# YufengJin/torch_renderer

Measured on AMD Instinct MI355X. Metric: frames/sec fwd+bwd, 512×512, ~6k-face mesh, batch=64; 1/2/4/8 MI355X, higher is better.
Workload: dtype f32; 1 GPU; cow (F=5856, V=2930), 512x512, 64 views/GPU, fwd+bwd: depth+silhouette+Phong RGB from one raster pass, grads to verts and per-view R,t; mesh=cow, H=512, W=512, views_per_gpu=64, global_views=64, parallelism=view-sharded x1

## Files before the change

torch_renderer_amd/csrc/mr_tile_raster.h:

```cpp
#pragma once

struct TileCols {
  float C0, C1;
  float omax;
};
MR_DEV TileCols tile_cols(int x0, int H, int W) {
  TileCols t;
  t.C1 = W > H ? 0.5f * (float)H : 0.5f * (float)W;
  t.C0 = 0.5f * (float)W - 0.5f - (float)x0;
  t.omax = (float)max(W, H) / (float)min(W, H);
  return t;
}
MR_DEV unsigned long long rect_mask(int rx0, int rx1, int ry0, int ry1) {
  const unsigned long long row = (2ull << rx1) - (1ull << rx0);
  const unsigned long long rows = (0x0101010101010101ull >> (8 * (7 - ry1))) & (~0ull << (8 * ry0));
  return row * rows;
}
MR_DEV unsigned long long tri_mask(const FaceRec& r, const float* ys, int rx0, int rx1, int ry0, int ry1,
                                   const TileCols& tc) {
  const float s = r.area > 0.0f ? 1.0f : -1.0f;
  float Gx[3], K[3], rA[3], ax[3], sC1[3], sC0[3];
  bool up[3];
  const float vx[3] = {r.x0, r.x1, r.x2}, vy[3] = {r.y0, r.y1, r.y2};
#pragma unroll
  for (int i = 0; i < 3; ++i) {
    const int a = (i + 1) % 3, b = (i + 2) % 3;
    const float dx = vx[b] - vx[a], dy = vy[b] - vy[a];
    const float A = s * dy;
    const float tol = 1e-6f * (fabsf(dx) + fabsf(dy)) * (tc.omax + fabsf(vx[a]) + fabsf(vy[a]));
    Gx[i] = s * dx;
    K[i] = Gx[i] * vy[a] + 2.0f * tol;
    up[i] = A >= 0.0f;
    rA[i] = A != 0.0f ? __builtin_amdgcn_rcpf(A) : 1e30f;
    ax[i] = vx[a];
    sC1[i] = up[i] ? -tc.C1 : tc.C1;
    sC0[i] = (up[i] ? tc.C0 : -tc.C0) + 0.02f;
  }
  unsigned long long m = 0;
#pragma unroll
  for (int ry = 0; ry < MR_TS; ++ry) {
    if (ry < ry0 || ry > ry1) continue;
    const float py = ys[ry];
    int hi = rx1, lo = rx0;
#pragma unroll
    for (int i = 0; i < 3; ++i) {
      const float T = fmaf(fmaf(Gx[i], py, -K[i]), rA[i], ax[i]);
      const float v = __builtin_amdgcn_fmed3f(fmaf(T, sC1[i], sC0[i]), -10.0f, 10.0f);
      const int h = (int)floorf(v);
      if (up[i]) hi = min(hi, h);
      else lo = max(lo, -h);
    }
    if (lo <= hi) m |= ((2ull << hi) - (1ull << lo)) << (8 * ry);
  }
  return m;
}

MR_DEV int kth_bit(unsigned long long m, int k) {
  const unsigned lo = (unsigned)m;
  const int clo = __popc(lo);
  const bool hi = k >= clo;
  unsigned x = hi ? (unsigned)(m >> 32) : lo;
  int pos = hi ? 32 : 0;
  k = hi ? k - clo : k;
#pragma unroll
  for (int sh = 16; sh >= 1; sh >>= 1) {
    const int c = __popc(x & ((1u << sh) - 1u));
    const bool go = k >= c;
    x = go ? x >> sh : x;
    k = go ? k - c : k;
    pos = go ? pos + sh : pos;
  }
  return pos;
}

MR_DEV bool frag_depth(const FaceRec& r, float x, float y, float pad, bool persp, bool clipb, bool fast, float& pz,
                       bool& inside) {
  if (x > r.xmax + pad || x < r.xmin - pad || y > r.ymax + pad || y < r.ymin - pad) return false;
  const float e0 = edge_fn(x, y, r.x1, r.y1, r.x2, r.y2);
  const float e1 = edge_fn(x, y, r.x2, r.y2, r.x0, r.y0);
  const float e2 = edge_fn(x, y, r.x0, r.y0, r.x1, r.y1);
  if (fast) {
    const bool inp = (e0 > 0.0f) & (e1 > 0.0f) & (e2 > 0.0f);
    const bool inn = (e0 < 0.0f) & (e1 < 0.0f) & (e2 < 0.0f);
    if (!(r.area > 0.0f ? inp : inn)) return false;
  }
  const float w0 = e0 / r.area, w1 = e1 / r.area, w2 = e2 / r.area;
  float c0, c1, c2, b0, b1, b2;
  if (persp) persp_fwd(w0, w1, w2, r.z0, r.z1, r.z2, c0, c1, c2);
  else { c0 = w0; c1 = w1; c2 = w2; }
  if (clipb) clip_fwd(c0, c1, c2, b0, b1, b2);
  else { b0 = c0; b1 = c1; b2 = c2; }
  pz = b0 * r.z0 + b1 * r.z1 + b2 * r.z2;
  if (pz < 0.0f) return false;
  inside = c0 > 0.0f && c1 > 0.0f && c2 > 0.0f;
  return true;
}

MR_DEV bool frag_keep(const FaceRec& r, float x, float y, float pad, float blur, bool persp, bool clipb,
                      bool fast, float& pz) {
  bool inside;
  if (!frag_depth(r, x, y, pad, persp, clipb, fast, pz, inside)) return false;
  if (!inside) {
    if (!(blur > 0.0f)) return false;
    if (pt_tri_dist(x, y, r) >= blur) return false;
  }
  return true;
}

#define MR_NONE 0x7fffffff

MR_DEV unsigned rec_code(int id, int64_t NF) {
  return id < NF ? 2u * (unsigned)id : 2u * (unsigned)(id - NF) + 1u;
}
MR_DEV int code_rec(unsigned code, int64_t NF) {
  return (code & 1u) ? (int)(NF + (code >> 1)) : (int)(code >> 1);
}
MR_DEV int rec_orig(int id, int64_t NF) { return id >= NF ? (int)(id - NF) : id; }

MR_DEV bool pair_keep(const FaceRec* __restrict__ recs, int64_t NF, int id, const FaceRec& r, float x, float y,
                      float pad, float blur, bool persp, bool clipb, int& cid, float& pz) {
  const bool second = id >= NF;
  const int oid = second ? (int)(id - NF) : (int)(id + NF);
  const FaceRec ro = recs[oid];
  const FaceRec& r1 = second ? ro : r;
  const FaceRec& r2 = second ? r : ro;
  const int id1 = second ? oid : id, id2 = second ? id : oid;
  FragEval e1, e2;
  const bool k1 = (r1.flags & FR_VALID) && eval_face(r1, x, y, pad, blur, persp, clipb, e1);
  const bool k2 = (r2.flags & FR_VALID) && eval_face(r2, x, y, pad, blur, persp, clipb, e2);
  if (k1 && k2) {
    const bool use2 = fabsf(e2.sdist) < fabsf(e1.sdist);
    cid = use2 ? id2 : id1;
    pz = use2 ? e2.pz : e1.pz;
    return true;
  }
  if (k1 || k2) {
    cid = k1 ? id1 : id2;
    pz = k1 ? e1.pz : e2.pz;
    return true;
  }
  return false;
}

struct StageRecs {
  float rec[16][64];
};
MR_DEV void stage_rec_put(StageRecs& S, int lane, const FaceRec& r) {
  const float* f = (const float*)&r;
#pragma unroll
  for (int i = 0; i < 16; ++i) S.rec[i][lane] = f[i];
}
MR_DEV FaceRec stage_rec_get(const StageRecs& S, int m) {
  FaceRec r;
  float* f = (float*)&r;
#pragma unroll
  for (int i = 0; i < 16; ++i) f[i] = S.rec[i][m];
  return r;
}
MR_DEV unsigned long long frag_key(float z, int f) {
  const unsigned zb = z == 0.0f ? 0u : __float_as_uint(z);
  return ((unsigned long long)zb << 32) | (unsigned)f;
}

struct FwdParams {
  int N, H, W, TX, T, K;
  float blur, bbox_pad;
  int persp, clipb;
  const int64_t* view_first;
  int64_t F;
  int64_t NF;
  const ClipRec* crec;
  const FaceRec* recs;
  const int* list;
  const int4* units;
  const int64_t* view_count;
  const int* cnt;
  const int* start;
  const int* vbase;
  int64_t list_cap;
  int mfpb;
  int fill;
  int emit_frag;
  int fill_first;
  int* ctr;
  unsigned long long* tkey;
  int* tdone;
  int* sface;
  const int* stile;
  int64_t* p2f;
  float* zbuf;
  float* bary;
  float* dists;
  ShadeParams S;
  const ShadeRec* srec;
  int out_flags;
  float* depth;
  float* sil;
  float* rgb;
  int32_t* p2f32;
  float4* frec;
  int* sgrp;
  uint8_t* sgpix;
  float isig;
  int4* sent;
  float4* spix;
  const int* sorder;
  int* sorder_ws;
  int4* units_ws2;
};

struct WaveStage {
  StageRecs rec;
  int id[64];
  int meta[64];
  int mark[64];
  unsigned long long key[64];
  unsigned long long cmask[64];
  float xs[MR_TS], ys[MR_TS];
};

struct Bg {
  float d, s, c[4];
};
template <int MODE>
MR_DEV Bg background(const FwdParams& P) {
  Bg b;
  b.d = b.s = -1.0f;
  b.c[0] = b.c[1] = b.c[2] = b.c[3] = -1.0f;
  if (MODE == 1) {
    PixGeom G;
    ShadeOut o;
    ShadeCache C;
    shade_fwd(P.S, 0, false, G, 0.f, 0.f, 0.f, 0.f, 0.f, o, C);
    b.d = o.depth;
    b.s = o.sil;
    b.c[0] = o.rgb[0]; b.c[1] = o.rgb[1]; b.c[2] = o.rgb[2]; b.c[3] = o.alpha;
  }
  return b;
}

template <int MODE, int CH>
MR_DEV void fill_chunk(const FwdParams& P, const Bg& b, int n, int c, bool vec) {
  const int lane = threadIdx.x & 63;
  const int64_t HW = (int64_t)P.H * P.W * (MODE == 0 ? P.K : 1);
  if (MODE == 0 && vec) {
    const int64_t q0 = (int64_t)c * 64;
    const int nq = (int)min((int64_t)64, HW / 4 - q0);
    if (nq <= 0) return;
    const int64_t pix = (int64_t)n * HW + 4 * q0;
    const float4 m1 = make_float4(-1.f, -1.f, -1.f, -1.f);
    const longlong2 l1 = make_longlong2(-1ll, -1ll);
    fill_words<2>((longlong2*)(P.p2f + pix), nq, lane, l1);
    fill_words<1>((float4*)(P.zbuf + pix), nq, lane, m1);
    fill_words<1>((float4*)(P.dists + pix), nq, lane, m1);
    fill_words<3>((float4*)(P.bary + pix * 3), nq, lane, m1);
  } else if (vec) {
    const int64_t g = (int64_t)c * 64 + lane;
    if (g >= HW / 4) return;
    const int64_t pix = (int64_t)n * HW + 4 * g;
    if (MODE == 0) {
      const float4 m1 = make_float4(-1.f, -1.f, -1.f, -1.f);
      longlong2* q = (longlong2*)(P.p2f + pix);
      q[0] = make_longlong2(-1ll, -1ll);
      q[1] = make_longlong2(-1ll, -1ll);
      *(float4*)(P.zbuf + pix) = m1;
      *(float4*)(P.dists + pix) = m1;
      float4* q3 = (float4*)(P.bary + pix * 3);
      q3[0] = m1; q3[1] = m1; q3[2] = m1;
    } else {
      if (P.out_flags & MR_OUT_DEPTH) *(float4*)(P.depth + pix) = make_float4(b.d, b.d, b.d, b.d);
      if (P.out_flags & MR_OUT_SIL) {
        if (P.out_flags & MR_OUT_SIL_RGBA) {
          float4* q = (float4*)(P.sil + pix * 4);
          const float4 v = make_float4(1.0f, 1.0f, 1.0f, b.s);
          q[0] = v; q[1] = v; q[2] = v; q[3] = v;
        } else {
          *(float4*)(P.sil + pix) = make_float4(b.s, b.s, b.s, b.s);
        }
      }
      if (P.p2f32) *(int4*)(P.p2f32 + pix) = make_int4(-1, -1, -1, -1);
      if (P.out_flags & MR_OUT_RGB) {
        float4* q = (float4*)(P.rgb + pix * CH);
        if (CH == 4) {
          const float4 v = make_float4(b.c[0], b.c[1], b.c[2], b.c[3]);
          q[0] = v; q[1] = v; q[2] = v; q[3] = v;
        } else {
          float r0 = b.c[0], g0 = b.c[1], b0 = b.c[2], r1 = r0, g1 = g0, b1 = b0, r2 = r0, g2 = g0, b2 = b0;
          asm volatile("" : "+v"(r1), "+v"(g1), "+v"(b1), "+v"(r2), "+v"(g2), "+v"(b2));
          q[0] = make_float4(r0, g0, b0, r1);
          q[1] = make_float4(g1, b1, r2, g2);
          q[2] = make_float4(b2, r0, g0, b0);
        }
      }
    }
  } else {
    const int64_t i = (int64_t)c * 64 + lane;
    if (i >= HW) return;
    const int64_t q = (int64_t)n * HW + i;
    if (MODE == 0) {
      P.p2f[q] = -1ll;
      P.zbuf[q] = -1.0f;
      P.dists[q] = -1.0f;
      for (int k = 0; k < 3; ++k) P.bary[q * 3 + k] = -1.0f;
    } else {
      if (P.out_flags & MR_OUT_DEPTH) P.depth[q] = b.d;
      if (P.out_flags & MR_OUT_SIL) {
        if (P.out_flags & MR_OUT_SIL_RGBA) *(float4*)(P.sil + q * 4) = make_float4(1.0f, 1.0f, 1.0f, b.s);
        else P.sil[q] = b.s;
      }
      if (P.p2f32) P.p2f32[q] = -1;
      if (P.out_flags & MR_OUT_RGB)
        for (int k = 0; k < CH; ++k) P.rgb[q * CH + k] = b.c[k];
    }
  }
}

MR_DEV void fill_frag_unlisted(const FwdParams& P, int n, int c) {
  const int lane = threadIdx.x & 63;
  const int64_t HW = (int64_t)P.H * P.W;
  const int64_t q0 = (int64_t)c * 64;
  const int nq = (int)min((int64_t)64, HW / 4 - q0);
  if (nq <= 0) return;
  bool listed = false;
  if (lane < nq) {
    const int p0 = (int)(4 * q0);
    int y = p0 / P.W, x = p0 - y * P.W + 4 * lane;
    while (x >= P.W) {
      x -= P.W;
      ++y;
    }
    listed = P.cnt[(int64_t)n * P.T + (y >> 3) * P.TX + (x >> 3)] > 0;
  }
  const unsigned long long lm = __ballot(listed);
  const int64_t pix = (int64_t)n * HW + 4 * q0;
  const float4 m1 = make_float4(-1.f, -1.f, -1.f, -1.f);
  longlong2* p2 = (longlong2*)(P.p2f + pix);
  float4* pz = (float4*)(P.zbuf + pix);
  float4* pd = (float4*)(P.dists + pix);
  float4* pb = (float4*)(P.bary + pix * 3);
#pragma unroll
  for (int k = 0; k < 2; ++k) {
    const int j = k * 64 + lane;
    if (j < 2 * nq && !((lm >> (j >> 1)) & 1ull)) p2[j] = make_longlong2(-1ll, -1ll);
  }
  if (lane < nq && !((lm >> lane) & 1ull)) {
    pz[lane] = m1;
    pd[lane] = m1;
  }
#pragma unroll
  for (int k = 0; k < 3; ++k) {
    const int j = k * 64 + lane;
    if (j < 3 * nq && !((lm >> (j / 3)) & 1ull)) pb[j] = m1;
  }
}

MR_DEV void fill_chunk_render_lc(const FwdParams& P, const Bg& b, int n, int c, int CH) {
  const int lane = threadIdx.x & 63;
  const int64_t HW = (int64_t)P.H * P.W;
  const int64_t q0 = (int64_t)c * 64;
  const int nq = (int)min((int64_t)64, HW / 4 - q0);
  if (nq <= 0) return;
  const int64_t pix = (int64_t)n * HW + 4 * q0;
  if (P.out_flags & MR_OUT_DEPTH) fill_words<1>((float4*)(P.depth + pix), nq, lane, make_float4(b.d, b.d, b.d, b.d));
  if (P.out_flags & MR_OUT_SIL) {
    if (P.out_flags & MR_OUT_SIL_RGBA) fill_words<4>((float4*)(P.sil + pix * 4), nq, lane, make_float4(1.0f, 1.0f, 1.0f, b.s));
    else fill_words<1>((float4*)(P.sil + pix), nq, lane, make_float4(b.s, b.s, b.s, b.s));
  }
  if (P.p2f32) fill_words<1>((int4*)(P.p2f32 + pix), nq, lane, make_int4(-1, -1, -1, -1));
  if (P.out_flags & MR_OUT_RGB) {
    float4* q = (float4*)(P.rgb + pix * CH);
    if (CH == 4) {
      fill_words<4>(q, nq, lane, make_float4(b.c[0], b.c[1], b.c[2], b.c[3]));
    } else {
      const float4 w0 = make_float4(b.c[0], b.c[1], b.c[2], b.c[0]);
      const float4 w1 = make_float4(b.c[1], b.c[2], b.c[0], b.c[1]);
      const float4 w2 = make_float4(b.c[2], b.c[0], b.c[1], b.c[2]);
#pragma unroll
      for (int k = 0; k < 3; ++k) {
        const int j = k * 64 + lane;
        if (j < 3 * nq) q[j] = (j % 3) == 0 ? w0 : (j % 3) == 1 ? w1 : w2;
      }
    }
  }
}

template <int MODE, int CH>
__global__ void __launch_bounds__(256) k_fill(FwdParams P) {
  const int gw = blockIdx.x * 4 + (threadIdx.x >> 6), G = gridDim.x * 4;
  const bool vec = (P.W & 3) == 0;
  const int64_t HW = (int64_t)P.H * P.W * (MODE == 0 ? P.K : 1);
  const int cpv = (int)(vec ? (HW / 4 + 63) / 64 : (HW + 63) / 64);
  const int nchunks = P.N * cpv;
  const Bg bg = background<MODE>(P);
#pragma unroll 1
  for (int c = gw; c < nchunks; c += G) {
    if (MODE == 1 && vec) fill_chunk_render_lc(P, bg, c / cpv, c - (c / cpv) * cpv, CH);
    else fill_chunk<MODE, CH>(P, bg, c / cpv, c - (c / cpv) * cpv, vec);
  }
}


#ifdef MR_XP_BV_STAMP
#define MR_XP_BV_WGS 4096
__device__ unsigned long long g_bv_stamp[MR_XP_BV_WGS * 8];
#endif
template <int MODE, int CH>
__global__ void __launch_bounds__(1024) k_bin_view(ViewBinParams P, FwdParams F) {
#ifdef MR_XP_BV_STAMP
  const unsigned long long xp_t0 = __builtin_amdgcn_s_memrealtime();
  const int xp_role = (int)blockIdx.x < P.nviews * P.bands ? 0 : (int)blockIdx.x < P.nviews * P.bands + P.nsrec_wg ? 1 : 2;
  struct XpEnd {
    unsigned long long t0;
    int role;
    __device__ ~XpEnd() {
      __syncthreads();
      const unsigned long long t1 = __builtin_amdgcn_s_memrealtime();
      const int i = (int)threadIdx.x;
      if (blockIdx.x < MR_XP_BV_WGS && i < 8)
        g_bv_stamp[(size_t)blockIdx.x * 8 + i] = i == 0 ? t0 : i == 1 ? t1 : i == 2 ? (unsigned long long)role
                                               : role == 0 ? g_bv_ph[i - 3] : 0ull;
    }
  } xp_end{xp_t0, xp_role};
#endif
  const int b = (int)blockIdx.x - P.nviews * P.bands - P.nsrec_wg;
  if (b < 0) {
    bin_view_body(P);
    return;
  }
  const int nbw = ((int)gridDim.x - P.nviews * P.bands - P.nsrec_wg) * 16;
  const bool vec = (F.W & 3) == 0;
  const int64_t HW = (int64_t)F.H * F.W * (MODE == 0 ? F.K : 1);
  const int cpv = (int)(vec ? (HW / 4 + 63) / 64 : (HW + 63) / 64);
  const Bg bg = background<MODE>(F);
  const int c0 = b * 16 + (int)(threadIdx.x >> 6);
  const int gn = nbw / cpv, gc = nbw - gn * cpv;
  int cn = c0 / cpv, cc = c0 - cn * cpv;
#pragma unroll 1
  for (int c = c0; c < F.fill_first; c += nbw) {
    fill_chunk<MODE, CH>(F, bg, cn, cc, vec);
    cn += gn;
    cc += gc;
    if (cc >= cpv) { cc -= cpv; ++cn; }
  }
}

__attribute__((noinline)) __device__ void raster_pair_rect(const FaceRec* __restrict__ recs, int64_t NF,
                                                           const StageRecs& srec, const int* sid, const float* xs,
                                                           const float* ys, unsigned long long* key, int lane,
                                                           int prect, float pad, float blur, bool persp, bool clipb) {
  const FaceRec r = stage_rec_get(srec, lane);
  const int id = sid[lane];
  for (int yy = (prect >> 6) & 7; yy <= ((prect >> 9) & 7); ++yy)
    for (int xx = prect & 7; xx <= ((prect >> 3) & 7); ++xx) {
      float pz;
      int cid;
      if (pair_keep(recs, NF, id, r, xs[xx], ys[yy], pad, blur, persp, clipb, cid, pz))
        atomicMin(&key[yy * MR_TS + xx], frag_key(pz, (int)rec_code(cid, NF)));
    }
}

#ifndef MR_TR_BGFIRST_FRAG
#define MR_TR_BGFIRST_FRAG 4
#endif
#ifndef MR_RASTER_WAVES
#define MR_RASTER_WAVES 4
#endif
template <int MODE, int CH, bool CLIP>
__global__ void __launch_bounds__(256, MR_RASTER_WAVES) k_tile_raster(FwdParams P) {
  __shared__ WaveStage stage[4];
  const int lane = threadIdx.x & 63;
  const int wave = __builtin_amdgcn_readfirstlane(threadIdx.x >> 6);
  WaveStage& S = stage[wave];
  const int nunits = P.ctr[CTR_UNITS];
  const float pad = P.bbox_pad, blur = P.blur;
  const bool persp = P.persp != 0, clipb = P.clipb != 0;
  const bool fast_ok = !(blur > 0.0f);
  const int H = P.H, W = P.W;
  const int gw = blockIdx.x * 4 + wave, G = gridDim.x * 4;
  const bool vec = (W & 3) == 0;
  const int64_t HW = (int64_t)H * W * (MODE == 0 ? P.K : 1);
  const int cpv = (int)(vec ? (HW / 4 + 63) / 64 : (HW + 63) / 64);
  const int nchunks = P.fill ? P.N * cpv : 0;
  const int parts = (gridDim.x & 7) == 0 ? 8 : 1;
  const int jw = (blockIdx.x / parts) * 4 + wave, Gp = (gridDim.x / parts) * 4;
  const int Cp = (nunits + parts - 1) / parts;
  const int ub = (blockIdx.x % parts) * Cp, ue = ub + Cp < nunits ? ub + Cp : nunits;
  const Bg bg = background<MODE>(P);
  int chunk = P.fill_first + gw;
  auto background_chunks = [&]() {
    const int gn = G / cpv, gc = G - gn * cpv;
    int cn = chunk / cpv, cc = chunk - cn * cpv;
    if (MODE == 0 && P.emit_frag) {
#pragma unroll 1
      for (; chunk < nchunks; chunk += G) {
        fill_frag_unlisted(P, cn, cc);
        cn += gn;
        cc += gc;
        if (cc >= cpv) { cc -= cpv; ++cn; }
      }
    } else {
#pragma unroll 1
      for (; chunk < nchunks; chunk += G) {
        fill_chunk<MODE, CH>(P, bg, cn, cc, vec);
        cn += gn;
        cc += gc;
        if (cc >= cpv) { cc -= cpv; ++cn; }
      }
    }
  };
  if (MODE == 0 && MR_TR_BGFIRST_FRAG > 0 &&
      (blockIdx.x + wave) % (MR_TR_BGFIRST_FRAG > 0 ? MR_TR_BGFIRST_FRAG : 1) == 0)
    background_chunks();
  const int lz = lane_zero();
  const int ulast = max(ue - 1, 0);
  int4 U1v = P.units[min(ub + jw, ulast) + lz];
  int4 U2v = P.units[min(ub + jw + Gp, ulast) + lz];
  int4 U3v = P.units[min(ub + jw + 2 * Gp, ulast) + lz];
  int id1 = P.list[(ub + jw < ue && U1v.y >= 0 && lane < U1v.z) ? U1v.y + lane : 0];
  int id2 = P.list[(ub + jw + Gp < ue && U2v.y >= 0 && lane < U2v.z) ? U2v.y + lane : 0];
  FaceRec r1 = load_rec(P.recs, (ub + jw < ue && U1v.y >= 0 && lane < U1v.z) ? id1 : 0);
#pragma unroll 1
  for (int u = ub + jw; u < ue; u += Gp) {
    const int4 U = make_int4(__builtin_amdgcn_readfirstlane(U1v.x), __builtin_amdgcn_readfirstlane(U1v.y),
                             __builtin_amdgcn_readfirstlane(U1v.z), __builtin_amdgcn_readfirstlane(U1v.w));
    const int id0 = id1;
    const int n = U.x / P.T, t = U.x - n * P.T;
    const int ty = t / P.TX, tx = t - ty * P.TX;
    const int x0 = tx * MR_TS, y0 = ty * MR_TS;
    const TileCols tc = tile_cols(x0, H, W);
    if (lane < MR_TS) S.xs[lane] = col_ndc(x0 + lane < W ? x0 + lane : W - 1, H, W);
    else if (lane < 2 * MR_TS) S.ys[lane - MR_TS] = row_ndc(y0 + lane - MR_TS < H ? y0 + lane - MR_TS : H - 1, H, W);
    S.key[lane] = MR_KEY_EMPTY;
    S.mark[lane] = -1;
    const bool ovf = U.y < 0;
    wave_lds_sync();
#pragma unroll 1
    for (int eb = 0; eb < U.z; eb += 64) {
      const int e = eb + lane;
      int prect = 0;
      unsigned long long cmask = 0;
      if (e < U.z) {
        int id;
        FaceRec r;
        if (ovf) {
          const int64_t vfirst = P.view_first ? P.view_first[n] : (int64_t)n * P.F;
          id = (int)(vfirst + e);
          r = P.recs[id];
        } else {
          id = id0;
          r = r1;
        }
        float bx0 = r.xmin, bx1 = r.xmax, by0 = r.ymin, by1 = r.ymax;
        bool bvalid = (r.flags & FR_VALID) != 0;
        if (CLIP && ovf && (r.flags & FR_PAIR)) {
          const FaceRec ro = P.recs[P.NF + id];
          if (ro.flags & FR_VALID) {
            bx0 = bvalid ? smin(bx0, ro.xmin) : ro.xmin;
            bx1 = bvalid ? smax(bx1, ro.xmax) : ro.xmax;
            by0 = bvalid ? smin(by0, ro.ymin) : ro.ymin;
            by1 = bvalid ? smax(by1, ro.ymax) : ro.ymax;
            bvalid = true;
          }
        }
        int cx0, cx1, cy0, cy1;
        ndc_range_to_pix(bx0 - pad, bx1 + pad, W, H, cx0, cx1);
        ndc_range_to_pix(by0 - pad, by1 + pad, H, W, cy0, cy1);
        cx0 = cx0 > x0 ? cx0 : x0;
        cx1 = cx1 < x0 + MR_TS - 1 ? cx1 : x0 + MR_TS - 1;
        cy0 = cy0 > y0 ? cy0 : y0;
        cy1 = cy1 < y0 + MR_TS - 1 ? cy1 : y0 + MR_TS - 1;
        if (bvalid && cx0 <= cx1 && cy0 <= cy1) {
          if (CLIP && (r.flags & FR_PAIR)) {
            prect = 0x1000 | (cx0 - x0) | ((cx1 - x0) << 3) | ((cy0 - y0) << 6) | ((cy1 - y0) << 9);
          } else {
            const int rx0 = cx0 - x0, rx1 = cx1 - x0, ry0 = cy0 - y0, ry1 = cy1 - y0;
            const bool tm = fast_ok && (r.flags & FR_FAST) &&
                            fmaxf(fmaxf(fabsf(r.xmin), fabsf(r.xmax)), fmaxf(fabsf(r.ymin), fabsf(r.ymax))) < 1e12f;
            cmask = tm ? tri_mask(r, S.ys, rx0, rx1, ry0, ry1, tc) : rect_mask(rx0, rx1, ry0, ry1);
          }
        }
        stage_rec_put(S.rec, lane, r);
        S.id[lane] = id;
      }
      if (eb == 0) {
        r1 = load_rec(P.recs, (u + Gp < ue && U2v.y >= 0 && lane < U2v.z) ? id2 : 0);
        id1 = id2;
        U1v = U2v;
        id2 = P.list[(u + 2 * Gp < ue && U3v.y >= 0 && lane < U3v.z) ? U3v.y + lane : 0];
        U2v = U3v;
        U3v = P.units[min(u + 3 * Gp, ulast) + lz];
      }
      const int np = __popcll(cmask);
      const int pincl = wave_incl_sum(np);
      const int pexcl = pincl - np;
      const int NP = __builtin_amdgcn_readlane(pincl, 63);
      S.meta[lane] = pexcl;
      S.cmask[lane] = cmask;
#pragma unroll 1
      for (int pb = 0; pb < NP; pb += 64) {
        wave_lds_sync();
        if (np > 0 && pexcl > pb && pexcl < pb + 64) S.mark[pexcl - pb] = lane;
        const unsigned long long own = __ballot(np > 0 && pexcl <= pb);
        const int straddle = 63 - __builtin_clzll(own);
        wave_lds_sync();
        int m = S.mark[lane];
        S.mark[lane] = -1;
        if (lane == 0) m = straddle;
        m = wave_incl_max(m);
        const int q = pb + lane;
        if (q < NP) {
          const int p = kth_bit(S.cmask[m], q - S.meta[m]);
          const int sx = p & 7, sy = p >> 3;
          const FaceRec r = stage_rec_get(S.rec, m);
          float pz;
          if (frag_keep(r, S.xs[sx], S.ys[sy], pad, blur, persp, clipb, fast_ok && (r.flags & FR_FAST), pz))
            atomicMin(&S.key[p], frag_key(pz, CLIP ? (int)rec_code(S.id[m], P.NF) : 2 * S.id[m]));
        }
      }
      if (CLIP && __builtin_expect(__ballot(prect != 0) != 0ull, 0)) {
        if (prect) raster_pair_rect(P.recs, P.NF, S.rec, S.id, S.xs, S.ys, S.key, lane, prect, pad, blur, persp, clipb);
      }
      wave_lds_sync();
    }
    unsigned long long k = S.key[lane];
    const int slot = U.w & 0x7fffffff;
    bool emit = true;
    if (U.w < 0) {
      unsigned long long* dst = P.tkey + (int64_t)slot * 64 + lane;
      atomicMin(dst, k);
      asm volatile("s_waitcnt vmcnt(0)" ::: "memory");
      int left = 0;
      if (lane == 0) left = __hip_atomic_fetch_add(&P.tdone[slot], -1, __ATOMIC_RELAXED, __HIP_MEMORY_SCOPE_AGENT);
      left = __builtin_amdgcn_readfirstlane(left);
      emit = left == 0;
      if (emit) k = atomicMin(dst, MR_KEY_EMPTY);
    }
    if (emit) {
      const unsigned code = (unsigned)(k & 0xffffffffull);
      const int px = x0 + (lane & 7), py = y0 + (lane >> 3);
      const bool hit = code != MR_NONE && px < W && py < H;
      const int rid = hit ? (CLIP ? code_rec(code, P.NF) : (int)(code >> 1)) : -1;
      if (MODE == 0 && P.emit_frag) {
        if (px < W && py < H) {
          const int64_t q = (int64_t)n * H * W + (int64_t)py * W + px;
          int64_t f = -1;
          float z = -1.0f, d = -1.0f, b0 = -1.0f, b1 = -1.0f, b2 = -1.0f;
          if (hit) {
            const FaceRec r = load_rec(P.recs, rid);
            FragEval ev;
            eval_face(r, S.xs[lane & 7], S.ys[lane >> 3], pad, blur, persp, clipb, ev);
            if (r.flags & FR_CLIP) clip_unconvert(P.crec[rid], ev.b0, ev.b1, ev.b2, ev.b0, ev.b1, ev.b2);
            f = rec_orig(rid, P.NF); z = ev.pz; d = ev.sdist; b0 = ev.b0; b1 = ev.b1; b2 = ev.b2;
          }
          P.p2f[q] = f;
          P.zbuf[q] = z;
          P.dists[q] = d;
          P.bary[3 * q + 0] = b0;
          P.bary[3 * q + 1] = b1;
          P.bary[3 * q + 2] = b2;
        }
      } else {
        P.sface[(int64_t)slot * 64 + lane] = rid;
      }
    }
    wave_lds_sync();
  }
  background_chunks();
}

__global__ void __launch_bounds__(256) k_shade_rec(ShadeParams S, int64_t F, ShadeRec* __restrict__ out) {
  const int64_t f = (int64_t)blockIdx.x * blockDim.x + threadIdx.x;
  if (f >= F) return;
  ShadeRec R;
  make_shade_rec(S, (uint32_t)f, R);
  out[f] = R;
}

__global__ void __launch_bounds__(256) k_setup_zero(const float* __restrict__ verts, int64_t V,
                                                    const int32_t* __restrict__ faces, const int32_t* __restrict__ ptr,
                                                    const int32_t* __restrict__ adj, float* __restrict__ vn,
                                                    float* __restrict__ vraw, int64_t vb, int* __restrict__ zero,
                                                    int64_t nzero) {
  if ((int64_t)blockIdx.x < vb) {
    const int64_t v = (int64_t)blockIdx.x * blockDim.x + threadIdx.x;
    if (v < V) vertex_normal(verts, faces, ptr, adj, v, vn, vraw);
    return;
  }
  const int64_t base = ((int64_t)blockIdx.x - vb) * 1024;
#pragma unroll
  for (int k = 0; k < 4; ++k) {
    const int64_t i = base + k * 256 + threadIdx.x;
    if (i < nzero) zero[i] = 0;
  }
}

MR_DEV void xcd_slot_range(int nslots, int wave, int& s0, int& step, int& end) {
  const int parts = (gridDim.x & 7) == 0 ? 8 : 1;
  const int per = (nslots + parts - 1) / parts;
  const int x = blockIdx.x % parts;
  const int b = x * per;
  end = b + per < nslots ? b + per : nslots;
  s0 = b + (int)(blockIdx.x / parts) * 4 + wave;
  step = (int)(gridDim.x / parts) * 4;
}

MR_DEV int sort_slot_pixels(int& f, int lane, int* lperm) {
  unsigned long long rem = ~0ull;
  int pos = 0, base = 0;
  while (rem) {
    const int l = (int)__builtin_ctzll(rem);
    const int key = __builtin_amdgcn_readlane(f, l);
    const unsigned long long m = __ballot(f == key);
    const int below = (int)__builtin_amdgcn_mbcnt_hi((unsigned)(m >> 32), __builtin_amdgcn_mbcnt_lo((unsigned)m, 0u));
    pos = f == key ? base + below : pos;
    base += __popcll(m);
    rem &= ~m;
  }
  lperm[pos] = lane;
  wave_lds_sync();
  const int src = lperm[lane];
  f = __builtin_amdgcn_ds_bpermute(src << 2, f);
  wave_lds_sync();
  return src;
}

template <int MODE, int CH>
__global__ void __launch_bounds__(256) k_shade(FwdParams P) {
  __shared__ int lperm[MODE == 1 ? 4 : 1][64];
  const int lane = threadIdx.x & 63;
  const int wave = __builtin_amdgcn_readfirstlane(threadIdx.x >> 6);
  const int nslots = P.ctr[CTR_SLOTS];
  if (nslots <= 0) return;
  const int64_t HW = (int64_t)P.H * P.W;
  int s0, G, send;
  xcd_slot_range(nslots, wave, s0, G, send);
  const int lz = lane_zero();
  const int slast = max(nslots - 1, 0);
  int sc = min(s0, slast);
  int gt_c = P.stile[sc + lz], f_c = P.sface[(int64_t)sc * 64 + lane];
  sc = min(s0 + G, slast);
  int gt_n = P.stile[sc + lz], f_n = P.sface[(int64_t)sc * 64 + lane];
  int p_c = MODE == 1 ? sort_slot_pixels(f_c, lane, lperm[wave]) : lane;
  FaceRec r_c = load_rec(P.recs, f_c < 0 ? 0 : f_c);
  for (int s = s0; s < send; s += G) {
    const int gt = __builtin_amdgcn_readfirstlane(gt_c);
    const int f = f_c, p = p_c;
    const FaceRec r = r_c;
    gt_c = gt_n;
    f_c = f_n;
    if (MODE == 1) p_c = sort_slot_pixels(f_c, lane, lperm[wave]);
    r_c = load_rec(P.recs, f_c < 0 ? 0 : f_c);
    sc = min(s + 2 * G, slast);
    gt_n = P.stile[sc + lz];
    f_n = P.sface[(int64_t)sc * 64 + lane];
    if (MODE == 1) {
      P.sgrp[(int64_t)s * 64 + lane] = f;
      P.sgpix[(int64_t)s * 64 + lane] = (uint8_t)p;
    }
    if (f < 0) continue;
    const int n = gt / P.T, t = gt - n * P.T;
    const int ty = t / P.TX, tx = t - ty * P.TX;
    const int px = tx * MR_TS + (p & 7), py = ty * MR_TS + (p >> 3);
    const int64_t q = n * HW + (int64_t)py * P.W + px;
    const int fo = rec_orig(f, P.NF);
    PixGeom G;
    if (MODE == 1) load_geom(P.srec, (uint32_t)(fo - n * P.F), G);
    FragEval ev;
    const bool hit = eval_face(r, col_ndc(px, P.H, P.W), row_ndc(py, P.H, P.W), P.bbox_pad, P.blur, P.persp,
                               P.clipb, ev);
    if (!hit) continue;
    if (r.flags & FR_CLIP) {
      const ClipRec cr = P.crec[f];
      clip_unconvert(cr, ev.b0, ev.b1, ev.b2, ev.b0, ev.b1, ev.b2);
    }
    if (MODE == 0) {
      P.p2f[q] = (int64_t)fo;
      P.zbuf[q] = ev.pz;
      P.dists[q] = ev.sdist;
      P.bary[3 * q + 0] = ev.b0;
      P.bary[3 * q + 1] = ev.b1;
      P.bary[3 * q + 2] = ev.b2;
    } else {
      P.frec[(int64_t)s * 64 + p] = make_float4(ev.b0, ev.b1, ev.b2, ev.sdist);
      ShadeOut o;
      ShadeCache C;
      shade_fwd(P.S, n, true, G, ev.b0, ev.b1, ev.b2, ev.pz, ev.sdist, o, C);
      if (P.out_flags & MR_OUT_DEPTH) P.depth[q] = o.depth;
      if (P.out_flags & MR_OUT_SIL) {
        if (P.out_flags & MR_OUT_SIL_RGBA) *(float4*)(P.sil + q * 4) = make_float4(1.0f, 1.0f, 1.0f, o.sil);
        else P.sil[q] = o.sil;
      }
      if (P.out_flags & MR_OUT_RGB) {
        P.rgb[q * CH + 0] = o.rgb[0];
        P.rgb[q * CH + 1] = o.rgb[1];
        P.rgb[q * CH + 2] = o.rgb[2];
        if (CH == 4) P.rgb[q * CH + 3] = o.alpha;
      }
      if (P.p2f32) P.p2f32[q] = fo;
    }
  }
}

template <int CH, int SPEC>
__global__ void __launch_bounds__(256) k_shade_render(FwdParams P) {
  __shared__ int lperm[4][64];
  const int lane = threadIdx.x & 63;
  const int wave = __builtin_amdgcn_readfirstlane(threadIdx.x >> 6);
  const int nslots = P.ctr[CTR_SLOTS];
  if (nslots <= 0) return;
  const int64_t HW = (int64_t)P.H * P.W;
  int s0, G, send;
  xcd_slot_range(nslots, wave, s0, G, send);
  const int lz = lane_zero();
  const int slast = max(nslots - 1, 0);
  int sc = min(s0, slast);
  int gt_c = P.stile[sc + lz], f_c = P.sface[(int64_t)sc * 64 + lane];
  sc = min(s0 + G, slast);
  int gt_n = P.stile[sc + lz], f_n = P.sface[(int64_t)sc * 64 + lane];
  int p_c = sort_slot_pixels(f_c, lane, lperm[wave]);
  FaceRec r_c = load_rec(P.recs, f_c < 0 ? 0 : f_c);
  const int of = SPEC ? (MR_OUT_DEPTH | MR_OUT_SIL | MR_OUT_RGB) : P.out_flags;
  int s_prev = -1, f_prev = -1, p_prev = 0, fo_prev = 0;
  bool w_prev = false;
  int64_t q_prev = 0;
  float4 fr_prev = make_float4(0.f, 0.f, 0.f, 0.f);
  ShadeOut o_prev;
  o_prev.depth = o_prev.sil = o_prev.alpha = 0.f;
  o_prev.rgb[0] = o_prev.rgb[1] = o_prev.rgb[2] = 0.f;
  auto store_prev = [&]() {
    if (s_prev < 0) return;
    P.sgrp[(int64_t)s_prev * 64 + lane] = f_prev;
    P.sgpix[(int64_t)s_prev * 64 + lane] = (uint8_t)p_prev;
    if (w_prev) {
      P.frec[(int64_t)s_prev * 64 + p_prev] = fr_prev;
      if (of & MR_OUT_DEPTH) P.depth[q_prev] = o_prev.depth;
      if (of & MR_OUT_SIL) {
        if (!SPEC && (of & MR_OUT_SIL_RGBA)) *(float4*)(P.sil + q_prev * 4) = make_float4(1.0f, 1.0f, 1.0f, o_prev.sil);
        else P.sil[q_prev] = o_prev.sil;
      }
      if (of & MR_OUT_RGB) {
        P.rgb[q_prev * CH + 0] = o_prev.rgb[0];
        P.rgb[q_prev * CH + 1] = o_prev.rgb[1];
        P.rgb[q_prev * CH + 2] = o_prev.rgb[2];
        if (CH == 4) P.rgb[q_prev * CH + 3] = o_prev.alpha;
      }
      if (!SPEC && P.p2f32) P.p2f32[q_prev] = fo_prev;
    }
  };
  for (int s = s0; s < send; s += G) {
    const int gt = __builtin_amdgcn_readfirstlane(gt_c);
    const int f = f_c, p = p_c;
    const FaceRec r = r_c;
    const int n = gt / P.T, t = gt - n * P.T;
    const int ty = t / P.TX, tx = t - ty * P.TX;
    const int px = tx * MR_TS + (p & 7), py = ty * MR_TS + (p >> 3);
    const int64_t q = n * HW + (int64_t)py * P.W + px;
    const int fo = f >= 0 ? (int)rec_orig(f, P.NF) : 0;
    PixGeom Gm;
    load_geom(P.srec, f >= 0 ? (uint32_t)(fo - n * P.F) : 0u, Gm);
    gt_c = gt_n;
    f_c = f_n;
    p_c = sort_slot_pixels(f_c, lane, lperm[wave]);
    r_c = load_rec(P.recs, f_c < 0 ? 0 : f_c);
    sc = min(s + 2 * G, slast);
    gt_n = P.stile[sc + lz];
    f_n = P.sface[(int64_t)sc * 64 + lane];
    store_prev();
    FragEval ev;
    const bool hit = f >= 0 && eval_face(r, col_ndc(px, P.H, P.W), row_ndc(py, P.H, P.W), P.bbox_pad, P.blur,
                                         P.persp, P.clipb, ev);
    ShadeOut o;
    o.depth = o.sil = o.alpha = 0.f;
    o.rgb[0] = o.rgb[1] = o.rgb[2] = 0.f;
    if (hit) {
      if (r.flags & FR_CLIP) {
        const ClipRec cr = P.crec[f];
        clip_unconvert(cr, ev.b0, ev.b1, ev.b2, ev.b0, ev.b1, ev.b2);
      }
      ShadeCache C;
      shade_fwd<SPEC>(P.S, n, true, Gm, ev.b0, ev.b1, ev.b2, ev.pz, ev.sdist, o, C);
    }
    s_prev = s;
    f_prev = f;
    p_prev = p;
    w_prev = hit;
    q_prev = q;
    fo_prev = fo;
    fr_prev = make_float4(ev.b0, ev.b1, ev.b2, ev.sdist);
    o_prev = o;
  }
  store_prev();
}

template <typename K>
static int resident_grid(K kernel, int threads, int fallback_per_cu) {
  int dev = 0, cus = 0, per = 0;
  (void)hipGetDevice(&dev);
  if (hipDeviceGetAttribute(&cus, hipDeviceAttributeMultiprocessorCount, dev) != hipSuccess || cus <= 0) cus = 256;
  if (hipOccupancyMaxActiveBlocksPerMultiprocessor(&per, kernel, threads, 0) != hipSuccess || per <= 0)
    per = fallback_per_cu;
  return cus * per;
}

static FwdParams make_fwd(const mr_raster_settings_t* s, const BinGeom& g, const RasterWS& w, int64_t N,
                          const int64_t* view_first, int64_t F, int64_t NF) {
  FwdParams P;
  memset(&P, 0, sizeof(P));
  P.N = (int)N; P.H = s->H; P.W = s->W; P.TX = g.TX; P.T = g.T; P.K = s->faces_per_pixel;
  P.blur = s->blur_radius;
  P.bbox_pad = sqrtf(s->blur_radius);
  P.persp = s->perspective_correct;
  P.clipb = s->clip_barycentric_coords;
  P.view_first = view_first; P.F = F; P.NF = NF; P.crec = w.crec;
  P.recs = w.recs; P.list = w.list; P.units = w.units; P.ctr = w.ctr; P.tkey = w.tkey;
  P.cnt = w.cnt; P.start = w.start; P.vbase = w.vbase; P.list_cap = g.list_cap; P.mfpb = g.mfpb;
  P.tdone = w.tdone; P.sface = w.sface; P.stile = w.stile;
  P.frec = w.frec;
  P.sgrp = w.sgrp;
  P.sgpix = w.sgpix;
  P.sorder_ws = w.sorder;
  P.units_ws2 = w.units2;
  return P;
}


#ifndef MR_UNIT_ORDER
#define MR_UNIT_ORDER 1
#endif
#ifndef MR_UNIT_ORDER_MIN_VIEWS
#define MR_UNIT_ORDER_MIN_VIEWS 16
#endif
MR_DEV int unit_key(const int4& U) { return U.y < 0 ? 0 : MR_UE + 1 - min(max(U.z, 1), MR_UE); }
__global__ void __launch_bounds__(1024) k_unit_order(const int4* __restrict__ units, const int* __restrict__ ctr,
                                                     int4* __restrict__ out) {
  __shared__ int hist[128];
  const int t = threadIdx.x, n = ctr[CTR_UNITS];
  const int per = (n + 7) / 8, b = (int)blockIdx.x * per, e = min(b + per, n);
  if (t < 128) hist[t] = 0;
  __syncthreads();
  for (int u = b + t; u < e; u += 1024) atomicAdd(&hist[unit_key(units[u])], 1);
  __syncthreads();
  if (t < 64) {
    const int x = hist[2 * t], y = hist[2 * t + 1];
    const int incl = wave_incl_sum(x + y);
    hist[2 * t] = b + incl - (x + y);
    hist[2 * t + 1] = b + incl - y;
  }
  __syncthreads();
  for (int u = b + t; u < e; u += 1024) {
    const int4 U = units[u];
    out[atomicAdd(&hist[unit_key(U)], 1)] = U;
  }
}

static int shade_grid(int64_t slots_cap, int resident) {
  const int sg = (int)(slots_cap / 4 + 1 < resident ? slots_cap / 4 + 1 : resident);
  return (sg + 7) / 8 * 8;
}

#ifndef MR_SHADE_RENDER
#define MR_SHADE_RENDER 1
#endif
template <int CH>
static int launch_shade_render(const FwdParams& P, int64_t slots_cap, hipStream_t st) {
  static int g0 = 0, g1 = 0;
  if (!g0) g0 = resident_grid(k_shade_render<CH, 0>, 256, 4);
  if (!g1) g1 = resident_grid(k_shade_render<CH, 1>, 256, 4);
  const bool spec = drop_in_shading(P.S, CH, P.out_flags) && !P.p2f32 &&
                    P.out_flags == (MR_OUT_DEPTH | MR_OUT_SIL | MR_OUT_RGB);
  const int sg = shade_grid(slots_cap, spec ? g1 : g0);
  return launch(KID_SHADE_RENDER, "k_shade_render", spec ? k_shade_render<CH, 1> : k_shade_render<CH, 0>, sg, 256, 0, st, P);
}

template <int MODE, int CH>
static int launch_raster_and_shade(FwdParams P, const BinGeom& g, int64_t N, hipStream_t st, bool clip) {
  P.fill = 1;
  static int rgrid = 0, rgrid_c = 0, sgrid = 0;
  if (!rgrid) rgrid = resident_grid(k_tile_raster<MODE, CH, false>, 256, 7);
  if (!rgrid_c) rgrid_c = resident_grid(k_tile_raster<MODE, CH, true>, 256, 7);
  if (!sgrid) sgrid = resident_grid(k_shade<MODE, CH>, 256, 6);
  if (MR_UNIT_ORDER && MODE == 1 && P.units_ws2 && N >= MR_UNIT_ORDER_MIN_VIEWS) {
    if (int rc = launch(KID_UNIT_ORDER, "k_unit_order", k_unit_order, 8, 1024, 0, st, P.units, P.ctr, P.units_ws2)) return rc;
    P.units = P.units_ws2;
  }
  if (int rc = launch(KID_TILE_RASTER, "k_tile_raster", clip ? k_tile_raster<MODE, CH, true> : k_tile_raster<MODE, CH, false>,
                      clip ? rgrid_c : rgrid, 256, 0, st, P))
    return rc;
  if (MODE == 0 && P.emit_frag) return MR_OK;
  const int64_t slots_cap = N * (int64_t)g.T;
  if (MODE == 1 && MR_SHADE_RENDER) return launch_shade_render<CH>(P, slots_cap, st);
  return launch(MODE == 0 ? KID_SHADE_FRAG : KID_SHADE_RENDER, "k_shade", k_shade<MODE, CH>, shade_grid(slots_cap, sgrid), 256, 0,
                st, P);
}

template <int CH>
static int launch_fill_and_shade(const FwdParams& P, int64_t slots_cap, hipStream_t st) {
  static int fgrid = 0, sgrid = 0;
  if (!fgrid) fgrid = resident_grid(k_fill<1, CH>, 256, 8);
  if (!sgrid) sgrid = resident_grid(k_shade<1, CH>, 256, 6);
  if (int rc = launch(KID_FILL_FRAG, "k_fill", k_fill<1, CH>, fgrid, 256, 0, st, P)) return rc;
  return launch(KID_SHADE_RENDER, "k_shade", k_shade<1, CH>, shade_grid(slots_cap, sgrid), 256, 0, st, P);
}
```

Measured before the change: 336,500 frames/s.

## Interleave background fill chunks into tile raster loop for render mode

Adds a BGQ variant of the tile raster kernel that writes one background fill chunk (depth, silhouette, packed RGB) per raster unit iteration, instead of leaving all background chunks to a loop after rasterization. The aim is to overlap the store-bound background fill with the compute- and latency-bound rasterization so the memory system stays busy while waves raster. It also adds an optional vmcnt-based pacing hook for background stores, disabled by default. The risk is extra stores and register pressure inside the hot raster loop, and leftover chunks are still handled by the existing tail fill.

```diff
diff --git a/torch_renderer_amd/csrc/mr_tile_raster.h b/torch_renderer_amd/csrc/mr_tile_raster.h
--- a/torch_renderer_amd/csrc/mr_tile_raster.h
+++ b/torch_renderer_amd/csrc/mr_tile_raster.h
@@ -384,6 +384,36 @@
   }
 }
 
+#ifndef MR_BG_INFLIGHT
+#define MR_BG_INFLIGHT 0
+#endif
+template <int MODE>
+MR_DEV void bg_pace() {
+  constexpr int cap = MR_BG_INFLIGHT;
+  if (cap > 0) {
+    constexpr int n = (MODE == 0 ? 7 : 5) * (cap > 0 ? cap - 1 : 0);
+    asm volatile("s_waitcnt vmcnt(%0)" ::"n"(n < 63 ? n : 63) : "memory");
+  }
+}
+
+MR_DEV void fill_chunk_static(const FwdParams& P, const Bg& b, int n, int c) {
+  const int lane = threadIdx.x & 63;
+  const int64_t HW = (int64_t)P.H * P.W;
+  const int64_t gi = (int64_t)c * 64 + lane, g = gi < HW / 4 ? gi : HW / 4 - 1;
+  const int64_t pix = (int64_t)n * HW + 4 * g;
+  *(float4*)(P.depth + pix) = make_float4(b.d, b.d, b.d, b.d);
+  *(float4*)(P.sil + pix) = make_float4(b.s, b.s, b.s, b.s);
+  float4* q = (float4*)(P.rgb + pix * 3);
+  float r0 = b.c[0], g0 = b.c[1], b0 = b.c[2], r1 = r0, g1 = g0, b1 = b0, r2 = r0, g2 = g0, b2 = b0;
+  asm volatile("" : "+v"(r1), "+v"(g1), "+v"(b1), "+v"(r2), "+v"(g2), "+v"(b2));
+  q[0] = make_float4(r0, g0, b0, r1);
+  q[1] = make_float4(g1, b1, r2, g2);
+  q[2] = make_float4(b2, r0, g0, b0);
+}
+static inline bool bg_static_outputs(const FwdParams& P) {
+  return P.out_flags == (MR_OUT_DEPTH | MR_OUT_SIL | MR_OUT_RGB) && !P.p2f32 && (P.W & 3) == 0;
+}
+
 template <int MODE, int CH>
 __global__ void __launch_bounds__(256) k_fill(FwdParams P) {
   const int gw = blockIdx.x * 4 + (threadIdx.x >> 6), G = gridDim.x * 4;
@@ -437,6 +467,7 @@
   int cn = c0 / cpv, cc = c0 - cn * cpv;
 #pragma unroll 1
   for (int c = c0; c < F.fill_first; c += nbw) {
+    bg_pace<MODE>();
     fill_chunk<MODE, CH>(F, bg, cn, cc, vec);
     cn += gn;
     cc += gc;
@@ -465,7 +496,10 @@
 #ifndef MR_RASTER_WAVES
 #define MR_RASTER_WAVES 4
 #endif
-template <int MODE, int CH, bool CLIP>
+#ifndef MR_TR_BG_INTERLEAVE
+#define MR_TR_BG_INTERLEAVE 1
+#endif
+template <int MODE, int CH, bool CLIP, bool BGQ = false>
 __global__ void __launch_bounds__(256, MR_RASTER_WAVES) k_tile_raster(FwdParams P) {
   __shared__ WaveStage stage[4];
   const int lane = threadIdx.x & 63;
@@ -493,6 +527,7 @@
     if (MODE == 0 && P.emit_frag) {
 #pragma unroll 1
       for (; chunk < nchunks; chunk += G) {
+        bg_pace<MODE>();
         fill_frag_unlisted(P, cn, cc);
         cn += gn;
         cc += gc;
@@ -501,6 +536,7 @@
     } else {
 #pragma unroll 1
       for (; chunk < nchunks; chunk += G) {
+        bg_pace<MODE>();
         fill_chunk<MODE, CH>(P, bg, cn, cc, vec);
         cn += gn;
         cc += gc;
@@ -511,6 +547,13 @@
   if (MODE == 0 && MR_TR_BGFIRST_FRAG > 0 &&
       (blockIdx.x + wave) % (MR_TR_BGFIRST_FRAG > 0 ? MR_TR_BGFIRST_FRAG : 1) == 0)
     background_chunks();
+  int qn = 0, qc = 0, qgn = 0, qgc = 0;
+  if constexpr (BGQ) {
+    qn = chunk / cpv;
+    qc = chunk - qn * cpv;
+    qgn = G / cpv;
+    qgc = G - qgn * cpv;
+  }
   const int lz = lane_zero();
   const int ulast = max(ue - 1, 0);
   int4 U1v = P.units[min(ub + jw, ulast) + lz];
@@ -589,6 +632,15 @@
         id2 = P.list[(u + 2 * Gp < ue && U3v.y >= 0 && lane < U3v.z) ? U3v.y + lane : 0];
         U2v = U3v;
         U3v = P.units[min(u + 3 * Gp, ulast) + lz];
+        if constexpr (BGQ) {
+          if (chunk < nchunks) {
+            fill_chunk_static(P, bg, qn, qc);
+            chunk += G;
+            qn += qgn;
+            qc += qgc;
+            if (qc >= cpv) { qc -= cpv; ++qn; }
+          }
+        }
       }
       const int np = __popcll(cmask);
       const int pincl = wave_incl_sum(np);
@@ -983,9 +1035,17 @@
     if (int rc = launch(KID_UNIT_ORDER, "k_unit_order", k_unit_order, 8, 1024, 0, st, P.units, P.ctr, P.units_ws2)) return rc;
     P.units = P.units_ws2;
   }
-  if (int rc = launch(KID_TILE_RASTER, "k_tile_raster", clip ? k_tile_raster<MODE, CH, true> : k_tile_raster<MODE, CH, false>,
-                      clip ? rgrid_c : rgrid, 256, 0, st, P))
-    return rc;
+  auto raster = clip ? k_tile_raster<MODE, CH, true> : k_tile_raster<MODE, CH, false>;
+  int grid = clip ? rgrid_c : rgrid;
+  if constexpr (MODE == 1 && CH == 3 && MR_TR_BG_INTERLEAVE != 0) {
+    if (!clip && bg_static_outputs(P)) {
+      static int qgrid = 0;
+      if (!qgrid) qgrid = resident_grid(k_tile_raster<1, 3, false, true>, 256, 7);
+      raster = k_tile_raster<1, 3, false, true>;
+      grid = qgrid;
+    }
+  }
+  if (int rc = launch(KID_TILE_RASTER, "k_tile_raster", raster, grid, 256, 0, st, P)) return rc;
   if (MODE == 0 && P.emit_frag) return MR_OK;
   const int64_t slots_cap = N * (int64_t)g.T;
   if (MODE == 1 && MR_SHADE_RENDER) return launch_shade_render<CH>(P, slots_cap, st);
```

New measurement: 345,400 frames/s, median of 6. +2.6%, better.
